# eaymerich/2015-RayTracing

Hardware: AMD Instinct MI355X
Metric: Msamples/sec (pixels x spp) at 1920x1080 (higher is better)
Workload: dtype f32; 1 GPU; A10 cornell.xml path trace 1920x1080, 256 spp (16x16 lens grid), 1 pass, 8 bounces, thin lens; one fused launch that resolves its own pixels (mirt_render_first_pass, no per-ray accumulator); width=1920, height=1080, rays_per_pixel=256, bounces=8, parallelism=rows/1, workload_key=cornell_1920x1080_r256_b8_n1

## Files before the change

2015-raytracing_amd/csrc/mirt_abi.cpp:

```cpp
#include "../../include/mirt.h"
#include "pt_launch.hpp"
#include "pt_post_check.hpp"
#include "pt_rows_plan.hpp"
#include "pt_view_plan.hpp"
#include "pt_set_guard.hpp"
#include "pt_stream_match.hpp"
#include "pt_upsample_taps.hpp"

#include <hip/hip_runtime.h>
#include <dlfcn.h>

#include <algorithm>
#include <cctype>
#include <cmath>
#include <cstdarg>
#include <cstdio>
#include <cstdlib>
#include <cstring>
#include <mutex>
#include <string>
#include <atomic>
#include <unordered_map>
#include <unordered_set>
#include <vector>

namespace {

constexpr size_t kRayBytes = 48, kPoiBytes = 64, kAcuBytes = 16;

thread_local std::string t_last_error = "";

enum HandleKind : uint8_t { H_CTX = 1, H_BUF, H_KERNEL, H_GRAPH, H_GROUP };
std::mutex g_live_mu;
std::unordered_map<const void*, HandleKind> g_live;
std::atomic<uint64_t> g_next_uid{1};

void live_add(const void* p, HandleKind k) { std::lock_guard<std::mutex> l(g_live_mu); g_live[p] = k; }
void live_del(const void* p) { std::lock_guard<std::mutex> l(g_live_mu); g_live.erase(p); }
bool live_is(const void* p, HandleKind k) {
    if (!p) return false;
    std::lock_guard<std::mutex> l(g_live_mu);
    auto it = g_live.find(p);
    return it != g_live.end() && it->second == k;
}

}

struct mirt_graph;
struct mirt_group;

using pt::ArgType; using pt::A_BUF; using pt::KernelId; using pt::KernelSpec; using pt::KArg; using pt::Enqueue; using pt::kKernels; using pt::arg_size; using pt::f2u_host;

struct mirt_ctx {
    int device = -1;
    hipStream_t own_stream = nullptr;
    hipStream_t stream = nullptr;
    std::string last_error;
    void* scratch = nullptr;
// ... 18 lines not shown
    size_t view_defer_bytes = 0;
    uint32_t view_defer_words = 0;
    bool inpass_resolve = true;
    bool last_pass_resolved = false;
    int force_exact = 0;
    bool profiling = false;
    hipEvent_t pe[3] = {nullptr, nullptr, nullptr};
    bool pe_valid = false;
    bool capturing = false;
    std::unordered_set<mirt_buf*> bufs;
    std::unordered_set<mirt_kernel*> kernels;
    std::unordered_set<mirt_graph*> graphs;
    mirt_group* group = nullptr;
    int fusion = 0;
    std::vector<Enqueue> pending;
    uint64_t fused_passes = 0;
    uint64_t guided_passes = 0;
    bool frame_fusion = false;
    uint64_t fused_frames = 0;
    uint64_t scratch_gen = 1, defer_gen = 1;
    struct Pin { mirt_buf* buf; uint64_t uid; uint64_t prep_gen; uint64_t version; bool content; };
    std::vector<Pin> cap_pins;
    bool cap_scratch = false, cap_defer = false;
};

static int flush_pending(mirt_ctx* ctx);
#define FLUSH_PENDING(ctx) do { if (!(ctx)->pending.empty()) { int _rc = flush_pending(ctx); if (_rc) return _rc; } } while (0)

struct mirt_graph {
    mirt_ctx* ctx = nullptr;
    hipGraph_t graph = nullptr;
    hipGraphExec_t exec = nullptr;
    std::vector<mirt_ctx::Pin> pins;
    uint64_t scratch_gen = 0, defer_gen = 0;
};

struct mirt_buf {
    mirt_ctx* ctx = nullptr;
    void* ptr = nullptr;
    size_t bytes = 0;
    bool owned = true;
    unsigned flags = 0;
    uint64_t uid = 0;
    uint64_t version = 1;
    uint64_t off_version = 0;
    uint32_t off_n = 0;
    uint32_t off_last = 0;
    uint32_t prep_count = 0;
    void* prep = nullptr;
    size_t prep_bytes = 0;
    uint64_t prep_version = 0;
    uint64_t prep_gen = 1;
    bool prep_sane = false;
};

struct mirt_kernel {
    mirt_ctx* ctx = nullptr;
    const KernelSpec* spec = nullptr;
    std::vector<KArg> args;
};

namespace {

bool live_has(const mirt_ctx* p) { return live_is(p, H_CTX); }
bool live_has(const mirt_buf* p) { return live_is(p, H_BUF); }
bool live_has(const mirt_kernel* p) { return live_is(p, H_KERNEL); }
bool live_has(const mirt_graph* p) { return live_is(p, H_GRAPH); }

int fail(mirt_ctx* ctx, int code, const char* fmt, ...) {
    char buf[512];
    va_list ap;
    va_start(ap, fmt);
    vsnprintf(buf, sizeof buf, fmt, ap);
    va_end(ap);
    t_last_error = buf;
    if (ctx && live_has(ctx)) ctx->last_error = buf;
    return code;
}

#define HIPCHK(ctx, expr)                                                                          \
    do {                                                                                           \
        hipError_t _e = (expr);                                                                    \
        if (_e != hipSuccess) return fail((ctx), MIRT_E_DEVICE, "%s: %s", #expr, hipGetErrorString(_e)); \
    } while (0)

#define NOT_WHILE_CAPTURING(ctx, what) \
    do { if ((ctx)->capturing) return fail((ctx), MIRT_E_ARG, "%s is not possible inside mirt_capture_begin/end: run the sequence once before recording it", (what)); } while (0)

void pin(mirt_ctx* ctx, const mirt_buf* b, bool content) {
    if (!ctx->capturing) return;
    for (auto& p : ctx->cap_pins)
        if (p.buf == b) { p.content = p.content || content; return; }
    ctx->cap_pins.push_back({const_cast<mirt_buf*>(b), b->uid, b->prep_gen, b->version, content});
}

int need(mirt_ctx* ctx, const char* what, const mirt_buf* b, uint64_t bytes) {
    if (!live_has(b)) return fail(ctx, MIRT_E_HANDLE, "%s: released or unknown buffer", what);
    if (b->ctx != ctx) return fail(ctx, MIRT_E_ARG, "%s: buffer belongs to another context", what);
    if ((uint64_t)b->bytes < bytes)
        return fail(ctx, MIRT_E_RANGE, "%s: buffer holds %zu bytes, launch needs %llu", what, b->bytes, (unsigned long long)bytes);
    pin(ctx, b, false);
    return MIRT_OK;
}

int check_grid(mirt_ctx* ctx, const char* what, mirt_buf* off, uint32_t n, const mirt_buf* prims, size_t prim_stride,
               const mirt_buf* normals, const mirt_buf* matid) {
    if (n == 0 || n > 1024) return fail(ctx, MIRT_E_ARG, "%s: n_slabs %u outside 1..1024", what, n);
    const uint64_t cells = (uint64_t)n * n * n;
    int rc = need(ctx, what, off, (cells + 1) * 4);
    if (rc) return rc;
    if (!off->owned || !(off->off_version == off->version && off->off_n == n)) {
        NOT_WHILE_CAPTURING(ctx, "validating a new cell-offset table");
        std::vector<uint32_t> h(cells + 1);
        HIPCHK(ctx, hipMemcpyAsync(h.data(), off->ptr, (cells + 1) * 4, hipMemcpyDeviceToHost, ctx->stream));
        HIPCHK(ctx, hipStreamSynchronize(ctx->stream));
        for (uint64_t i = 0; i < cells; ++i) {
            if (h[i] > h[i + 1]) return fail(ctx, MIRT_E_DATA, "%s: cell offsets decrease at cell %llu", what, (unsigned long long)i);
            if (n > 1 && h[i + 1] - h[i] >= pt::kMaxCellSlots)
                return fail(ctx, MIRT_E_RANGE, "%s: cell %llu holds %u slots (a cell of a grid holds at most %u)", what, (unsigned long long)i, h[i + 1] - h[i], pt::kMaxCellSlots - 1u);
        }
        off->off_version = off->version;
        off->off_n = n;
        off->off_last = h[cells];
    }
    pin(ctx, off, true);
    const uint64_t count = off->off_last;
    rc = need(ctx, what, prims, count * prim_stride);
    if (rc) return rc;
    if (normals && (rc = need(ctx, what, normals, count * prim_stride))) return rc;
    if (matid && (rc = need(ctx, what, matid, count * 4))) return rc;
    return MIRT_OK;
}

int ensure_scratch(mirt_ctx* ctx, size_t bytes);

int ensure_prepared(mirt_ctx* ctx, mirt_buf* pb, uint32_t count) {
    const size_t bytes = pt::prepared_bytes(count);
    if (pb->owned && pb->prep_version == pb->version && pb->prep_count == count && pb->prep_bytes >= bytes && (pb->prep || !bytes)) { pin(ctx, pb, true); return MIRT_OK; }
    NOT_WHILE_CAPTURING(ctx, "preparing a new triangle buffer");
    if (pb->prep && pb->prep_bytes < bytes) { HIPCHK(ctx, hipStreamSynchronize(ctx->stream)); HIPCHK(ctx, hipFree(pb->prep)); pb->prep = nullptr; pb->prep_bytes = 0; pb->prep_gen++; }
    if (bytes && !pb->prep) { HIPCHK(ctx, hipMalloc(&pb->prep, bytes)); pb->prep_bytes = bytes; pb->prep_gen++; }
    int rc = ensure_scratch(ctx, 16);
    if (rc) return rc;
    uint32_t insane = 0;
    HIPCHK(ctx, hipMemsetAsync(ctx->scratch, 0, 4, ctx->stream));
    pt::launch_prepTriangles(ctx->stream, pb->ptr, pb->prep, count, (uint32_t*)ctx->scratch);
    HIPCHK(ctx, hipMemcpyAsync(&insane, ctx->scratch, 4, hipMemcpyDeviceToHost, ctx->stream));
    HIPCHK(ctx, hipStreamSynchronize(ctx->stream));
    pb->prep_sane = insane == 0;
    pb->prep_version = pb->version;
    if (pb->prep_count != count) pb->prep_gen++;
    pb->prep_count = count;
    return MIRT_OK;
}

int ensure_scratch(mirt_ctx* ctx, size_t bytes) {
    if (ctx->capturing) ctx->cap_scratch = true;
    if (ctx->scratch_bytes >= bytes) return MIRT_OK;
    NOT_WHILE_CAPTURING(ctx, "growing the scratch buffer");
    if (ctx->scratch) { HIPCHK(ctx, hipStreamSynchronize(ctx->stream)); HIPCHK(ctx, hipFree(ctx->scratch)); ctx->scratch = nullptr; ctx->scratch_bytes = 0; }
    ctx->scratch_gen++;
    HIPCHK(ctx, hipMalloc(&ctx->scratch, bytes));
    ctx->scratch_bytes = bytes;
    return MIRT_OK;
}

int grow_and_clear(mirt_ctx* ctx, void*& ptr, size_t& have, size_t need_bytes) {
    if (have < need_bytes) {
        if (ptr) { HIPCHK(ctx, hipStreamSynchronize(ctx->stream)); HIPCHK(ctx, hipFree(ptr)); ptr = nullptr; have = 0; }
        HIPCHK(ctx, hipMalloc(&ptr, need_bytes));
        have = need_bytes;
    }
    HIPCHK(ctx, hipMemsetAsync(ptr, 0, need_bytes, ctx->stream));
    return MIRT_OK;
}

void add_range(std::vector<pt::PostRange>& in, const mirt_buf* b) { if (b && live_has(b)) in.push_back({(uint64_t)(uintptr_t)b->ptr, (uint64_t)b->bytes, true}); }
void add_geometry_ranges(std::vector<pt::PostRange>& in, const mirt_pass_desc* d) {
    const auto add_grid = [&in](const mirt_grid* g) { if (g) { add_range(in, g->prims); add_range(in, g->normals); add_range(in, g->matid); add_range(in, g->cell_offsets); } };
    add_grid(d->spheres); add_grid(d->triangles);
    for (uint32_t m = 0; m < d->n_meshes; ++m) add_grid(&d->meshes[m]);
}

void free_buf(mirt_buf* buf, bool ctx_alive) {
    mirt_ctx* ctx = buf->ctx;
    live_del(buf);
    if (ctx_alive) {
        ctx->bufs.erase(buf);
        if ((buf->owned && buf->ptr) || buf->prep) {
            (void)hipSetDevice(ctx->device);
            (void)hipStreamSynchronize(ctx->stream);
        }
        if (buf->owned && buf->ptr) (void)hipFree(buf->ptr);
        if (buf->prep) (void)hipFree(buf->prep);
    }
    delete buf;
}
void free_kernel(mirt_kernel* k, bool ctx_alive) {
    live_del(k);
    if (ctx_alive) k->ctx->kernels.erase(k);
    delete k;
}
// ... 847 lines not shown
            if ((rc = need(ctx, "pixels", A(K::pixels), npx * 4))) return rc;
            if ((rc = need(ctx, "rays", A(K::rays), npx * kRayBytes))) return rc;
            if (S.id == pt::K_a04_initTrace) pt::launch_frame_initTrace(st, false, A(K::pixels)->ptr, A(K::fcam), A(K::rays)->ptr, nullptr, g0, g1);
            else if (S.id == pt::K_a07_initTrace) pt::launch_frame_initTrace(st, true, A(K::pixels)->ptr, A(K::fcam), A(K::rays)->ptr, A(pt::a07_initTrace::bound), g0, g1);
            else {
                namespace M4 = pt::a04_meshTrace; namespace MM = pt::a07_molTrace; namespace MT = pt::a07_meshTrace;
                pt::FrameArgs F = {};
                memcpy(F.cam, A(K::fcam), 64); F.pixels = A(K::pixels)->ptr; F.rays = A(K::rays)->ptr; F.gx = g0; F.gy = g1;
                if (S.id == pt::K_a04_meshTrace) rc = frame_a04_mesh(ctx, S.name, A(M4::t_size), A(M4::t_pos), A(M4::t_normal), A(M4::t_mindex), A(M4::m_color), F);
                else if (S.id == pt::K_a07_molTrace) rc = frame_a07_mol(ctx, S.name, A(MM::bound), A(MM::n_slabs), A(MM::slab_size), A(MM::s_atoms), F);
                else rc = frame_a07_mesh(ctx, S.name, A(MT::bound), A(MT::n_slabs), A(MT::slab_size), A(MT::t_pos), A(MT::t_normal), F);
                if (rc) return rc;
                pt::launch_frame_stage(st, F, S.id == pt::K_a04_meshTrace ? pt::FS_A04 : S.id == pt::K_a07_molTrace ? pt::FS_MOL : pt::FS_MESH);
            }
            break;
        }
        default:
            return fail(ctx, MIRT_E_NAME, "kernel not implemented");
    }
    HIPCHK(ctx, hipGetLastError());
    return MIRT_OK;
}

static int fill_grid(mirt_ctx* ctx, const char* what, const mirt_grid* g, bool tri, bool per_prim_matid, pt::GridArgs* o) {
    if (!g->prims || !g->cell_offsets) return fail(ctx, MIRT_E_ARG, "%s: null geometry buffer", what);
    if (tri && !g->normals) return fail(ctx, MIRT_E_ARG, "%s: triangles need a normal buffer", what);
    if (per_prim_matid && !g->matid) return fail(ctx, MIRT_E_ARG, "%s: needs a per-primitive material buffer", what);
    int rc = check_grid(ctx, what, g->cell_offsets, g->n_slabs, g->prims, tri ? 48 : 16, tri ? g->normals : nullptr,
                        per_prim_matid ? g->matid : nullptr);
    if (rc) return rc;
    o->prims = g->prims->ptr;
    o->kind = tri ? pt::KIND_TRIANGLES : pt::KIND_SPHERES;
    if (tri) {
        mirt_buf* pb = g->prims;
        if ((rc = ensure_prepared(ctx, pb, g->cell_offsets->off_last))) return rc;
        o->prims = pb->prep ? pb->prep : pb->ptr;
        o->pnorm = pb->prep && g->cell_offsets->off_last <= pt::kLdsTriMax ? (const char*)pb->prep + pt::prepared_planes_offset(g->cell_offsets->off_last) : nullptr;
    }
    o->normals = tri ? g->normals->ptr : nullptr;
    o->matid = per_prim_matid ? g->matid->ptr : nullptr;
    o->off = g->cell_offsets->ptr;
    memcpy(o->bound, g->bounds, sizeof o->bound);
    o->n = g->n_slabs;
    o->mesh_matid = g->mesh_matid;
    o->nslots = g->cell_offsets->off_last;
    const pt::SetGuard v = pt::set_guard(g->bounds, g->n_slabs, !tri || g->prims->prep_sane);
    o->fast_ok = v.fast_ok;
    o->walk_ok = v.walk_ok;
    o->exit_is_far_face = v.exit_is_far_face;
    o->exit_far_axes = v.exit_far_axes;
    memcpy(o->exit_up, v.exit_up, sizeof o->exit_up);
    memcpy(o->delta, v.delta, sizeof o->delta);
    memcpy(o->rdelta, v.rdelta, sizeof o->rdelta);
    return MIRT_OK;
}

static pt::PassRequest pass_request(const mirt_ctx* ctx, const mirt_pass_desc* d, const PassOpts& o) {
    pt::PassRequest r;
    r.rpp = d->rays_per_pixel;
    r.npix = (uint64_t)(d->nrows ? d->nrows : d->height) * d->width;
    r.passes = o.passes;
    r.fresh = o.fresh;
    r.has_acu = d->acu != nullptr;
    r.has_pixel = d->pixel != nullptr;
    r.has_radiance = d->radiance != nullptr;
    r.every = o.every;
    r.inpass_resolve = ctx->inpass_resolve;
    return r;
}

static int fill_sets(mirt_ctx* ctx, const char* fn, const mirt_pass_desc* d, pt::FusedArgs& A);
static int fill_shading(mirt_ctx* ctx, const mirt_pass_desc* d, pt::FusedArgs& A, bool with_material);
static int pass_setup(mirt_ctx* ctx, const char* fn, const mirt_pass_desc* d, bool guides, pt::FusedArgs& A, bool with_material = true) {
    if (!d || d->struct_size != sizeof(mirt_pass_desc)) return fail(ctx, MIRT_E_ARG, "%s: descriptor size mismatch", fn);
    if (!d->width || !d->height || !d->rays_per_pixel) return fail(ctx, MIRT_E_ARG, "%s: empty image", fn);
    {
        const uint32_t k = (uint32_t)std::sqrt((double)d->rays_per_pixel);
        const uint32_t kk = (k + 1) * (k + 1) == d->rays_per_pixel ? k + 1 : k;
        if (kk * kk != d->rays_per_pixel)
            return fail(ctx, MIRT_E_ARG, "%s: rays_per_pixel %u is not a square (the lens grid is k x k, A10 code.js:540)", fn, d->rays_per_pixel);
    }
    if (!guides && d->n_lights > MIRT_MAX_LIGHTS) return fail(ctx, MIRT_E_ARG, "%s: %u lights > %d (enqueue the kernels one by one instead)", fn, d->n_lights, MIRT_MAX_LIGHTS);
    if (d->n_meshes > MIRT_MAX_MESHES) return fail(ctx, MIRT_E_ARG, "%s: %u meshes > %d (enqueue the kernels one by one instead)", fn, d->n_meshes, MIRT_MAX_MESHES);
    if ((!guides && d->n_lights && !d->lights) || (d->n_meshes && !d->meshes)) return fail(ctx, MIRT_E_ARG, "%s: null light/mesh array", fn);
    if (!guides && !d->pass_index) return fail(ctx, MIRT_E_ARG, "%s: pass_index is 1-based", fn);
    const uint32_t cols = f2u_host(d->cam[14]), rows = f2u_host(d->cam[15]);
    if (cols != d->width || rows != d->height) return fail(ctx, MIRT_E_ARG, "%s: camera says %ux%u, descriptor %ux%u", fn, cols, rows, d->width, d->height);
    const uint32_t nrows = d->nrows ? d->nrows : d->height;
    if (d->row0 >= d->height || nrows > d->height - d->row0) return fail(ctx, MIRT_E_ARG, "%s: row tile [%u,+%u) outside the image", fn, d->row0, nrows);
    const uint64_t npix = (uint64_t)nrows * d->width;
    const uint64_t nrays = npix * d->rays_per_pixel;
    if (nrays > 0xFFFFFF00ull) return fail(ctx, MIRT_E_ARG, "%s: %llu rays in one tile (the kernels index a tile's rays with 32 bits); split the rows over more launches", fn, (unsigned long long)nrays);
    HIPCHK(ctx, hipSetDevice(ctx->device));

    memset(&A, 0, sizeof A);
    memcpy(A.cam, d->cam, sizeof A.cam);
    memcpy(A.bound, d->scene_bounds, sizeof A.bound);
    A.focal_length = d->focal_length; A.lens_rad = d->lens_rad;
    A.width = d->width; A.height = d->height; A.rpp = d->rays_per_pixel;
    A.row0 = d->row0; A.nrows = nrows; A.bounces = d->bounces;
    A.n_lights = guides ? 0u : d->n_lights;
    int rc;
    if ((rc = fill_sets(ctx, fn, d, A))) return rc;
    return fill_shading(ctx, d, A, with_material);
}

// ... 1391 lines not shown
```

2015-raytracing_amd/csrc/pt_direct.hpp:

```cpp
#pragma once
#include "pt_closest.hpp"

#ifndef PT_SKIP_DARK_SHADOWS
#define PT_SKIP_DARK_SHADOWS 1
#endif
namespace pt {

template <int STRIDE, bool ATTE_LDS>
struct ParkT : ClosestHooks {
    static constexpr bool kAtteLds = ATTE_LDS;
    static constexpr int kP = ATTE_LDS ? 7 : 4, kN = kP + 3;
    float* base;
    PT_DEV void put(int w, float v) const { base[w * STRIDE] = v; }
    PT_DEV float get(int w) const { return base[w * STRIDE]; }
    PT_DEV void acc_add(float x, float y, float z) const {
        put(0, get(0) + x); put(1, get(1) + y); put(2, get(2) + z); put(3, get(3) + 1.0f);
    }
    PT_DEV void put_pn(const Poi& q) const { put(kP, q.p.x); put(kP + 1, q.p.y); put(kP + 2, q.p.z); put(kN, q.n.x); put(kN + 1, q.n.y); put(kN + 2, q.n.z); }
    PT_DEV void get_pn(Poi& q) const { q.p = mk3(get(kP), get(kP + 1), get(kP + 2)); q.n = mk3(get(kN), get(kN + 1), get(kN + 2)); }
};
typedef ParkT<256, true> Park;

template <bool FAST, int GRIDS, class PARK>
PT_DEV void direct_all(const FusedArgs& A, Poi& poi, int32_t& seed, float4& acc, const PARK& park, bool& defer) {
    const float4* material = (const float4*)A.material;
    for (uint32_t l = 0; l < A.n_lights; ++l) {
        const LightArgs& L = A.lights[l];
        const bool path = poi.matId >= 0;
        bool dark = false;
        Ray sh;
        sh.o = mk3(0.0f, 0.0f, 0.0f);
        sh.d = mk3(0.0f, 0.0f, 0.0f);
        sh.mint = PT_INF;
        sh.maxt = PT_INF;
        if (path) {
#if PT_PARK_LDS
            if (PT_PARK_PN_FOR(GRIDS)) park.get_pn(poi);
#endif
            sh = shadow_ray(poi, ld3(L.shadow), ld3(L.shadow + 3), ld3(L.shadow + 6), L.shadow[9], seed);
#if PT_SKIP_DARK_SHADOWS
            if (GRIDS) {
                const float cosx = cl_clamp(dot3(sh.d, poi.n), 0.0f, 1.0f);
                const float cosy = cl_clamp(dot3(neg3(sh.d), ld3(L.scene + 3)), 0.0f, 1.0f);
                const float r = len3(sub3(poi.p, ld3(L.scene)));
                const float fin = L.scene[9] * 0.0f + L.scene[6] * 0.0f + L.scene[7] * 0.0f + L.scene[8] * 0.0f;
                dark = (cosx * cosy == 0.0f) & (r * r > 0.0f) & (fin == 0.0f);
            }
            if (FAST && !dark) defer = defer || !ray_guard(sh);
#else
            if (FAST) defer = defer || !ray_guard(sh);
#endif
        }
        const RayRcp rr = ray_rcp<FAST>(sh);
        for (uint32_t s = 0; s < A.n_sets; ++s) {
            const GridArgs& S = A.sets[s];
            const bool live = path && !dark && !(sh.mint == sh.maxt);
            Hit ch;
            bool walked = false;
            if (!GRIDS || S.n == 1u) {
                if (live) {
                    pt_count(PC_BOX_TESTS); pt_count(PC_BOX_LANES, true);
                    const BoxHit bh = inter_aabb_t<FAST, !PT_AABB_UNSIGNED_ZERO>(sh, rr, set_box(S));
                    if (bh.v) {
                        ch = (S.kind == KIND_SPHERES) ? trace_cell1<SPHERES, true, TRI_A10, FAST, true>(sh, rr, bh, S) : trace_cell1<TRIANGLES, true, TRI_A10, FAST, true, PT_LANE_LISTS_FOR(FAST, GRIDS)>(sh, rr, bh, S);
                        walked = true;
                    }
                }
            } else if (S.kind == KIND_TRIANGLES) {
                BoxHit bh = {};
                if (live) bh = inter_aabb_t<FAST, true>(sh, rr, set_box(S));
                walked = live && bh.v;
                ch = trace_dda_coop<COOP_ANY, FAST, GRIDS == 1>(walked, sh, rr, bh, S, defer);
            } else if (live) {
                const BoxHit bh = inter_aabb_t<FAST, true>(sh, rr, set_box(S));
                if (bh.v) {
                    ch = trace_dda<SPHERES, true, TRI_A10, FAST, GRIDS == 1>(sh, bh, S, defer);
                    walked = true;
                }
            }
            if (!walked) continue;
            sh.maxt = ch.t;
            if (ch.idx != UINT32_MAX) sh.mint = ch.t;
        }
        if (!path || (uint32_t)poi.matId >= A.nmat) continue;
        pt_count(PC_SHADE); pt_count(PC_SHADE_LANES, true);
        float4 c4 = material[poi.matId];
#if PT_PARK_LDS
        if (PT_PARK_PN_FOR(GRIDS)) park.get_pn(poi);
        if (PARK::kAtteLds) poi.atte = mk3(park.get(4), park.get(5), park.get(6));
        f3 c = shade_vertex(poi, sh, mk3(c4.x, c4.y, c4.z), ld3(L.scene), ld3(L.scene + 3), ld3(L.scene + 6), L.scene[9]);
        if (PARK::kAtteLds) { park.put(4, poi.atte.x); park.put(5, poi.atte.y); park.put(6, poi.atte.z); }
        park.acc_add(c.x, c.y, c.z);
#else
        f3 c = shade_vertex(poi, sh, mk3(c4.x, c4.y, c4.z), ld3(L.scene), ld3(L.scene + 3), ld3(L.scene + 6), L.scene[9]);
        acc.x += c.x; acc.y += c.y; acc.z += c.z; acc.w += 1.0f;
#endif
    }
}

}
```

2015-raytracing_amd/csrc/pt_launch.hpp:

```cpp
#pragma once
#include <hip/hip_runtime.h>
#include <stdint.h>

#include "pt_pass_plan.hpp"

namespace pt {

enum { KIND_SPHERES = 0, KIND_TRIANGLES = 1 };

void launch_sizeof(hipStream_t s, bool ray, uint32_t* out);
void launch_initAcu(hipStream_t s, void* acu, uint32_t total, uint32_t gsz);
void launch_lensDraws(hipStream_t s, void* seeds, void* uv, uint32_t cols, uint32_t rows, uint32_t gx, uint32_t gy,
                      uint32_t row0, uint32_t nrows);
void launch_initTrace(hipStream_t s, void* rays, void* pois, const void* uv, const float* bound, const float* cam,
                      float focal, float lens_rad, uint32_t rpp, uint32_t gx, uint32_t gy);
void launch_bouncePaths(hipStream_t s, const void* pois, void* rays, void* seeds, uint32_t total, uint32_t gsz);
void launch_lightRender(hipStream_t s, void* pois, void* rays, void* acu, const float* light, uint32_t total, uint32_t gsz);
void launch_initShadowTrace(hipStream_t s, void* shadow, const void* pois, uint32_t total, const float* light, void* seeds, uint32_t gsz);
void launch_closest(hipStream_t s, int kind, uint32_t total, void* pois, void* rays, const void* prims, const void* normals,
                    const void* matid, uint32_t mesh_matid, const void* off, const float* bound, uint32_t n, uint32_t exit_far, uint32_t gsz);
void launch_anyhit(hipStream_t s, int kind, uint32_t total, void* shadow, const void* prims, const void* off, const float* bound,
                   uint32_t n, uint32_t exit_far, uint32_t gsz);
void launch_sceneRender(hipStream_t s, void* acu, void* pois, const void* shadow, const void* material, uint32_t nmat,
                        const float* light, uint32_t total, uint32_t gsz);
void launch_copyToPixel(hipStream_t s, void* pixel, const void* acu, float m, uint32_t pixels, uint32_t rpp, uint32_t gsz, void* radiance);
void launch_numerics(hipStream_t s, int op, const void* a, const void* b, void* out, uint64_t n);
void launch_divCheck(hipStream_t s, int mode, uint64_t seed, uint64_t count, void* out16);
void launch_seedFill(hipStream_t s, void* seeds, uint64_t first, uint64_t count, uint32_t base);

constexpr int kMaxLights = 8;
constexpr int kMaxMeshes = 16;

constexpr uint32_t kNoLds = 0xFFFFFFFFu;
constexpr uint32_t kLdsOffWords = 4096;
constexpr uint32_t kLdsTriMax = 96;
struct GridArgs {
    const void* prims;
    const void* pnorm;
    const void* normals;
    const void* matid;
    const void* off;
    float bound[8];
    uint32_t n;
    uint32_t mesh_matid;
    uint32_t kind;
    uint32_t fast_ok;
    uint32_t lds_off;
    float delta[3], rdelta[3];
    uint32_t nslots;
    uint32_t exit_far_axes;
    float exit_up[3];
    uint32_t walk_ok;
    uint32_t exit_is_far_face;
};
struct LightArgs {
    float shadow[16];
    float scene[16];
    float light[16];
};
struct FusedArgs {
    float cam[16];
    float bound[8];
    float focal_length, lens_rad;
    uint32_t width, height, rpp;
    uint32_t row0, nrows;
    uint32_t bounces;
    uint32_t n_sets, n_lights;
    GridArgs sets[2 + kMaxMeshes];
    LightArgs lights[kMaxLights];
    const void* material;
    uint32_t nmat;
    int32_t* seeds;
    void* acu;
    const void* uv;
    uint32_t fresh;
    void* pixel;
    void* radiance;
    float res_m;
    uint32_t resolve;
    uint32_t seg_off;
    uint32_t seg_len;
    uint32_t seg_pitch;
    uint32_t passes;
    uint32_t every;
    uint32_t pass_index;
    const void* carry;
    void* guide_nh;
    void* guide_ad;
};
inline bool all_sets_fast_ok(const FusedArgs& a) { for (uint32_t i = 0; i < a.n_sets; ++i) if (!a.sets[i].fast_ok) return false; return true; }
void launch_fused(hipStream_t s, const FusedArgs& a, bool fast, uint32_t* defer_mask, const uint32_t* redo_mask, uint32_t redo_words);
bool fused_fast_available();
bool fused_has_grids(const FusedArgs& a);
bool fused_multipass_default(const FusedArgs& a);
void launch_deferCount(hipStream_t s, const uint32_t* mask, uint32_t words, uint32_t* count);
void launch_guides(hipStream_t s, const FusedArgs& a, bool fast, void* normal_hits, void* albedo_depth, uint32_t* defer_mask, const uint32_t* redo_mask);
void launch_rays(hipStream_t s, const FusedArgs& a, bool fast, const void* rays, uint32_t count, void* hits, uint32_t* sets, uint8_t* occluded,
                 uint32_t* defer_mask, const uint32_t* redo_mask);
void launch_ao(hipStream_t s, const FusedArgs& a, bool fast, uint32_t samples, float radius, float bias, void* ao_out, uint32_t* defer_mask, const uint32_t* redo_mask);
void launch_radiance(hipStream_t s, const FusedArgs& a, bool fast, const void* rays, uint32_t count, uint32_t samples, uint32_t flags, int32_t* seeds, void* radiance,
                     uint32_t* defer_mask, const uint32_t* redo_mask);
struct ViewArgs {
    uint32_t model;
    uint32_t width, height;
    uint32_t k;
    uint32_t row0, nrows;
// ... 99 lines not shown
```

2015-raytracing_amd/csrc/pt_trace.hpp:

```cpp
#pragma once
#include "pt_device.hpp"
#include "pt_launch.hpp"
#include "pt_windows.hpp"

#ifndef PT_UNROLL_UNIFORM
#define PT_UNROLL_UNIFORM 1
#endif

namespace pt {

#ifndef PT_COUNT
#define PT_COUNT 0
#endif
enum PtCounter { PC_WAVES = 0, PC_SEGMENTS, PC_SEG_LANES, PC_Q_CLOSEST, PC_Q_CLOSEST_LANES, PC_SWEEP_CLOSEST, PC_TRIPS_CLOSEST, PC_TRIP_LANES_CLOSEST,
                 PC_Q_SHADOW, PC_Q_SHADOW_LANES, PC_SWEEP_SHADOW, PC_TRIPS_SHADOW, PC_TRIP_LANES_SHADOW,
                 PC_SPH_Q_CLOSEST, PC_SPH_Q_CLOSEST_LANES, PC_SPH_TESTS_CLOSEST, PC_SPH_ROOTS_CLOSEST, PC_SPH_Q_SHADOW, PC_SPH_Q_SHADOW_LANES, PC_SPH_TESTS_SHADOW, PC_SPH_ROOTS_SHADOW,
                 PC_BOX_TESTS, PC_BOX_LANES, PC_SHADE, PC_SHADE_LANES, PC_BOUNCE, PC_BOUNCE_LANES,
                 PC_GRID_WALKS, PC_GRID_WANT_LANES = PC_GRID_WALKS + 2, PC_GRID_PHASES = PC_GRID_WALKS + 4, PC_GRID_A_STEPS = PC_GRID_WALKS + 6,
                 PC_GRID_A_LANE_STEPS = PC_GRID_WALKS + 8, PC_GRID_ROUNDS = PC_GRID_WALKS + 10, PC_GRID_PAIRS = PC_GRID_WALKS + 12, PC_COUNT = 48 };
#if PT_COUNT
static __device__ unsigned long long pt_counters[PC_COUNT];
__device__ __forceinline__ void pt_count(int i, bool lanes = false, unsigned long long n = 1ull) {
    const unsigned long long m = __builtin_amdgcn_ballot_w64(true);
    const unsigned me = __builtin_amdgcn_mbcnt_hi(~0u, __builtin_amdgcn_mbcnt_lo(~0u, 0u));
    if (me == (unsigned)__builtin_ctzll(m)) atomicAdd(&pt_counters[i], lanes ? (unsigned long long)__builtin_popcountll(m) : n);
}
#else
__device__ __forceinline__ void pt_count(int, bool = false, unsigned long long = 1ull) {}
#endif

struct Hit { uint32_t idx; float t, beta, gamma; };

PT_DEV f3 interp_normal(const float4* nn, float beta, float gamma) {
    const float w = 1.0f - beta - gamma;
    return norm3(fma3(gamma, ld3(nn[2]), fma3(w, ld3(nn[0]), scl3(beta, ld3(nn[1])))));
}

#define PT_CONST_AS __attribute__((address_space(4)))
typedef float pt_v4f __attribute__((ext_vector_type(4)));
typedef float pt_v16f __attribute__((ext_vector_type(16)));
PT_DEV float4 ldc4(const void* base, size_t idx) {
    const pt_v4f v = ((const pt_v4f PT_CONST_AS*)base)[idx];
    return make_float4(v.x, v.y, v.z, v.w);
}
PT_DEV uint32_t ldc_u32(const void* base, size_t idx) { return ((const uint32_t PT_CONST_AS*)base)[idx]; }

#ifndef PT_GUARD_INT
#define PT_GUARD_INT 1
#endif
enum TriRule { TRI_A10 = 0, TRI_A07 = 1, TRI_A04 = 2 };
#ifndef PT_UNIFORM_CULL
#define PT_UNIFORM_CULL 0
#endif
#ifndef PT_SPHERE_WAVE_SKIP
#define PT_SPHERE_WAVE_SKIP 1
#endif
template <int RULE = TRI_A10, bool FAST = false, bool WAVE_CULL = false>
PT_DEV bool tri_test(f3 o, f3 d, float cmin, float cmax, const float4 A, const float4 B, const float4 C,
                     float& t_out, float& beta_out, float& gamma_out) {
    const f3 p0 = mk3(A.x, A.y, A.z), e1 = mk3(B.x, B.y, B.z), e2 = mk3(C.x, C.y, C.z), n = mk3(A.w, B.w, C.w);
    float div = dot3(n, d);
    if (WAVE_CULL && __builtin_amdgcn_ballot_w64(!(div <= 0)) == 0ull) { t_out = 0.0f; beta_out = 0.0f; gamma_out = 0.0f; return false; }
    float idiv;
    if (FAST) idiv = rcp_refined(div);
    else idiv = rcp_plain(div);
    f3 s = sub3(o, p0);
    float beta = dot3(cross3(s, d), e2) * idiv;
    float gamma = dot3(cross3(s, e1), d) * idiv;
    float gb = gamma + beta;
    float t = dot3(cross3(s, e2), e1) * -idiv;
    int ok = !(div <= 0);
    ok &= !(beta < 0.0f) & !(beta > 1.0f);
// ... 192 lines not shown
    const bool fwd = d >= 0;
    a.dslab = fwd ? 1 : -1;
    a.limit = fwd ? (int)n : -1;
    a.dt = div_exact3_anyzero(delta, cl_fabs(d), cl_fabs(rd));
    const float xnext = cl_fma((float)(a.slab + (fwd ? 1 : 0)), delta, lo);
    const float num1 = xnext - o;
    a.tnext = div_exact3_anyzero(num1, d, rd);
    defer = ((int)defer | (int)!((int)num_window(num0) & (int)num_window(num1))) != 0;
    return a;
}

PT_DEV uint32_t sign_word(float w) {
    uint32_t r;
    asm("v_ashrrev_i32 %0, 31, %1" : "=v"(r) : "v"(w));
    return r;
}

extern __shared__ __attribute__((aligned(16))) uint32_t pt_lds_dyn[];

PT_DEV Box set_box_of(const GridArgs& S) {
    Box b;
    b.lo = mk3(S.bound[0], S.bound[1], S.bound[2]);
    b.hi = mk3(S.bound[4], S.bound[5], S.bound[6]);
    return b;
}
template <bool FAST>
PT_DEV float cell1_exit(const Ray& ray, const RayRcp& rr, const BoxHit& bh, const GridArgs& S) {
    float tn[3];
    if (S.exit_is_far_face) {
        tn[0] = bh.tfx; tn[1] = bh.tfy; tn[2] = bh.tfz;
#if !PT_PLAIN_DIV
    } else if (FAST) {
        const float tf[3] = {bh.tfx, bh.tfy, bh.tfz}, up[3] = {S.exit_up[0], S.exit_up[1], S.exit_up[2]};
        const float oo[3] = {ray.o.x, ray.o.y, ray.o.z}, dd[3] = {ray.d.x, ray.d.y, ray.d.z}, rc[3] = {rr.x, rr.y, rr.z};
#pragma unroll
        for (int k = 0; k < 3; ++k) {
            const float q = div_exact3_anyzero(up[k] - oo[k], dd[k], rc[k]);
            tn[k] = (((S.exit_far_axes >> k) & 1u) != 0u || !(dd[k] >= 0.0f)) ? tf[k] : q;
        }
#endif
    } else {
        const float lo[3] = {S.bound[0], S.bound[1], S.bound[2]}, hi[3] = {S.bound[4], S.bound[5], S.bound[6]};
        const float oo[3] = {ray.o.x, ray.o.y, ray.o.z}, dd[3] = {ray.d.x, ray.d.y, ray.d.z};
#pragma unroll
        for (int k = 0; k < 3; ++k) {
            float delta = (hi[k] - lo[k]) / 1.0f;
            float xnext = lo[k] + (float)((dd[k] >= 0) ? 1 : 0) * delta;
            tn[k] = (xnext - oo[k]) / dd[k];
        }
    }
    return cl_min(cl_min(tn[0], tn[1]), tn[2]);
}

template <int KIND, bool ANY, int RULE = TRI_A10, bool FAST = false, bool FLAG_ONLY = false, bool LANES = false>
PT_DEV Hit trace_cell1(const Ray& ray, const RayRcp& rr, const BoxHit& bh, const GridArgs& S) {
    Hit ch;
    ch.idx = UINT32_MAX;
    ch.t = ray.maxt;
    ch.beta = 0.0f;
    ch.gamma = 0.0f;
    SphereRay sr;
    if (KIND == SPHERES) sr = sphere_ray<FAST>(ray.d);
    const float cmin = bh.tmin;
    const float cmax = cell1_exit<FAST>(ray, rr, bh, S);
    const uint32_t begin = __builtin_amdgcn_readfirstlane(ldc_u32(S.off, 0));
    const uint32_t end = __builtin_amdgcn_readfirstlane(ldc_u32(S.off, 1));
    bool done = false;
    if (LANES && KIND == TRIANGLES && FAST && RULE == TRI_A10 && S.lds_off != kNoLds && begin == 0u) {
        const pt_v16f PT_CONST_AS* pn = (const pt_v16f PT_CONST_AS*)((const char PT_CONST_AS*)S.pnorm + 64);
        const uint32_t lds_bytes = S.lds_off * 4u;
        const float o1 = __builtin_fabsf(ray.o.x) + __builtin_fabsf(ray.o.y) + __builtin_fabsf(ray.o.z);
        const float hi_p = __builtin_fmaxf(__builtin_fminf(cmax, ray.maxt) * 1.00000095367431640625f, 0x1p-100f);
        const float lo_m = cmin * 0.99999904632568359375f;
        pt_count(ANY ? PC_Q_SHADOW : PC_Q_CLOSEST); pt_count(ANY ? PC_Q_SHADOW_LANES : PC_Q_CLOSEST_LANES, true);
        for (uint32_t c0 = 0u; c0 < end; c0 += 32u) {
            const uint32_t groups = ldc_u32(S.pnorm, c0 >> 5);
            const pt_v16f PT_CONST_AS* g = pn + ldc_u32(S.pnorm, 4u + (c0 >> 5));
            const float Mu = cl_fma(__uint_as_float(ldc_u32(S.pnorm, 8u + (c0 >> 5))), o1, __uint_as_float(ldc_u32(S.pnorm, 12u + (c0 >> 5))));
            uint32_t cand = 0u;
            auto verdict = [&](float div, float sn, uint32_t mask, uint32_t back) {
                const float sp = sn + Mu, sm = sn - Mu;
                const float w = __builtin_fminf(__builtin_fminf(div, cl_fma(hi_p, div, sp)), -cl_fma(lo_m, div, sm));
                cand |= mask & ~sign_word(w);
                if (back != 0u) {
                    asm volatile("" ::: "memory");
                    const float wb = __builtin_fminf(__builtin_fminf(-div, -cl_fma(hi_p, div, sm)), cl_fma(lo_m, div, sp));
                    cand |= back & ~sign_word(wb);
                }
            };
#define PT_AXIS_GROUPS(SHIFT, OA, DA)                                                                                   \
            for (uint32_t i = 0; i < ((groups >> SHIFT) & 255u); ++i, ++g) {                                            \
                const pt_v16f v = *g;                                                                                   \
                _Pragma("unroll") for (int k = 0; k < 4; ++k) {                                                         \
                    const uint32_t mask = __float_as_uint(v[4 * k + 2]), back = __float_as_uint(v[4 * k + 3]);          \
                    if ((mask | back) == 0u) continue;                 \
                    asm volatile("" ::: "memory");                                                                      \
                    pt_count(ANY ? PC_SWEEP_SHADOW : PC_SWEEP_CLOSEST);                                                 \
                    verdict(v[4 * k + 1] * (DA), v[4 * k + 1] * ((OA) - v[4 * k]), mask, back);                         \
                }                                                                                                       \
            }
            PT_AXIS_GROUPS(0, ray.o.x, ray.d.x)
            PT_AXIS_GROUPS(8, ray.o.y, ray.d.y)
            PT_AXIS_GROUPS(16, ray.o.z, ray.d.z)
#undef PT_AXIS_GROUPS
            for (uint32_t i = 0; i < groups >> 24; ++i, ++g) {
                const pt_v16f v = *g;
#pragma unroll
                for (int k = 0; k < 2; ++k) {
                    const uint32_t mask = __float_as_uint(v[8 * k + 4]), back = __float_as_uint(v[8 * k + 5]);
                    if ((mask | back) == 0u) continue;
                    asm volatile("" ::: "memory");
                    pt_count(ANY ? PC_SWEEP_SHADOW : PC_SWEEP_CLOSEST);
                    const float div = dot3(mk3(v[8 * k], v[8 * k + 1], v[8 * k + 2]), ray.d);
                    const float sn = cl_fma(v[8 * k + 2], ray.o.z, cl_fma(v[8 * k + 1], ray.o.y, cl_fma(v[8 * k], ray.o.x, -v[8 * k + 3])));
                    verdict(div, sn, mask, back);
                }
            }
            if (ANY && done) cand = 0u;
            while (cand != 0u) {
                pt_count(ANY ? PC_TRIPS_SHADOW : PC_TRIPS_CLOSEST); pt_count(ANY ? PC_TRIP_LANES_SHADOW : PC_TRIP_LANES_CLOSEST, true);
                const uint32_t k = (uint32_t)__builtin_clz(cand);
                cand &= ~(0x80000000u >> k);
                const uint32_t i = c0 + k;
                const float4* __restrict__ q = (const float4*)((const char*)pt_lds_dyn + (lds_bytes + __umul24(i, 48u)));
                float ti, b, gm;
                const bool hit = tri_test_nn(ray.o, ray.d, cmin, cmax, q[0], q[1], q[2], ti, b, gm);
                if (ANY && FLAG_ONLY) {
                    if (hit && ti < ray.maxt) { done = true; cand = 0u; }
                    continue;
                }
                const bool better = (int)hit & (int)(ti < ch.t);
                ch.t = better ? ti : ch.t;
                ch.idx = better ? i : ch.idx;
                ch.beta = better ? b : ch.beta;
                ch.gamma = better ? gm : ch.gamma;
                if (ANY && better) { done = true; cand = 0u; }
            }
            if (ANY && __builtin_amdgcn_ballot_w64(!done) == 0ull) break;
        }
        if (ANY && FLAG_ONLY && done) ch.idx = 0u;
        return ch;
    }
    if (KIND == SPHERES) { pt_count(ANY ? PC_SPH_Q_SHADOW : PC_SPH_Q_CLOSEST); pt_count(ANY ? PC_SPH_Q_SHADOW_LANES : PC_SPH_Q_CLOSEST_LANES, true); }
    const pt_v4f PT_CONST_AS* p = (const pt_v4f PT_CONST_AS*)S.prims + (size_t)begin * (KIND == SPHERES ? 1u : 3u);
#if PT_UNROLL_UNIFORM > 1
#pragma unroll PT_UNROLL_UNIFORM
#endif
    for (uint32_t i = begin; i < end; ++i, p += (KIND == SPHERES ? 1 : 3)) {
        float ti, b = 0.0f, gm = 0.0f;
        bool hit;
        if (KIND == SPHERES) {
            pt_count(ANY ? PC_SPH_TESTS_SHADOW : PC_SPH_TESTS_CLOSEST);
            hit = sph_test<FAST, PT_SPHERE_WAVE_SKIP != 0, ANY ? PC_SPH_ROOTS_SHADOW : PC_SPH_ROOTS_CLOSEST>(ray.o, ray.d, sr, cmin, cmax, ldc4((const void*)p, 0), ti);
        } else {
            hit = tri_test<RULE, FAST, PT_UNIFORM_CULL != 0>(ray.o, ray.d, cmin, cmax, ldc4((const void*)p, 0), ldc4((const void*)p, 1), ldc4((const void*)p, 2), ti, b, gm);
        }
// ... 115 lines not shown
```

profiles/trip_counts.py:

```python
#!/usr/bin/env python3
import ctypes as C
import json
import os
import sys

import numpy as np

ROOT = os.path.dirname(os.path.dirname(os.path.abspath(__file__)))
sys.path.insert(0, ROOT)
import __graft_entry__ as graft

NAMES = ["waves", "segments", "seg_lanes", "q_closest", "q_closest_lanes", "sweep_closest", "trips_closest", "trip_lanes_closest",
         "q_shadow", "q_shadow_lanes", "sweep_shadow", "trips_shadow", "trip_lanes_shadow",
         "sph_q_closest", "sph_q_closest_lanes", "sph_tests_closest", "sph_roots_closest", "sph_q_shadow", "sph_q_shadow_lanes", "sph_tests_shadow", "sph_roots_shadow",
         "box_tests", "box_lanes", "shade", "shade_lanes", "bounce", "bounce_lanes",
         "grid_walks_closest", "grid_walks_shadow", "grid_want_lanes_closest", "grid_want_lanes_shadow", "grid_phases_closest", "grid_phases_shadow",
         "grid_a_steps_closest", "grid_a_steps_shadow", "grid_a_lane_steps_closest", "grid_a_lane_steps_shadow", "grid_rounds_closest", "grid_rounds_shadow",
         "grid_pairs_closest", "grid_pairs_shadow"]


def main():
    graft.load_package()
    from raytracing_amd.pyhost import mirt, render, scene
    name = sys.argv[1] if len(sys.argv) > 1 else "cornell"
    w, h, rpp, bounces = (int(x) for x in (sys.argv[2:6] if len(sys.argv) > 5 else (1920, 1080, 16, 8)))
    if name == "cornell":
        base = scene.PackedScene(open(os.path.join(ROOT, "tests", "golden", "scene_cornell_1920x1080_r256.json")).read())
    else:
        fx = np.load(os.path.join(ROOT, "tests", "golden", name + ".npz"))
        base = scene.PackedScene(bytes(fx["scene_json"]).decode())
    sc = base.resized(w, h, rpp)
    lib = mirt.lib()
    if not hasattr(lib, "mirt_debug_counters"):
        raise SystemExit("this libmirt.so is not a counting build (-DPT_COUNT=1)")
    ctx = mirt.Context(0)
    fr = render.FusedRenderer(ctx, sc, keep_acu=False)
    out = (C.c_ulonglong * 48)()
    lib.mirt_debug_counters(None, 1)
    fr.execute_render(bounces=bounces, fresh=True)
    ctx.finish()
    lib.mirt_debug_counters(out, 0)
    c = dict(zip(NAMES, list(out)))
    waves = c["waves"]
    print(json.dumps({"scene": name, "width": w, "height": h, "rpp": rpp, "bounces": bounces, "counters": c}))
    print(f"{'counter':28s} {'total':>14s} {'per wave':>10s}")
    for k in NAMES:
        print(f"{k:28s} {c[k]:14d} {c[k] / waves:10.2f}")
    fr.release()
    ctx.destroy()


if __name__ == "__main__":
    main()
```

Before: 5530 Msamples/s.

## Skip axis-aligned plane tests for shadow rays inside a precomputed empty gap

Adds a host-side analysis of the axis-aligned triangle planes of a single-cell triangle set. It computes a conservative slab on each axis that no axis-aligned plane crosses, with error margins. In the shadow path, a wave whose rays all have segments inside that slab skips the AABB test and all axis-aligned plane groups, and tests only the general-plane groups. This adds a plane readback at prep time and a per-ray gap test with a wave ballot, at the risk of extra divergence or of the test rarely passing.

```diff
diff --git a/2015-raytracing_amd/csrc/mirt_abi.cpp b/2015-raytracing_amd/csrc/mirt_abi.cpp
--- a/2015-raytracing_amd/csrc/mirt_abi.cpp
+++ b/2015-raytracing_amd/csrc/mirt_abi.cpp
@@ -4,6 +4,7 @@
 #include "pt_rows_plan.hpp"
 #include "pt_view_plan.hpp"
 #include "pt_set_guard.hpp"
+#include "pt_shadow_gap.hpp"
 #include "pt_stream_match.hpp"
 #include "pt_upsample_taps.hpp"
 
@@ -128,6 +129,8 @@
     uint64_t prep_version = 0;
     uint64_t prep_gen = 1;
     bool prep_sane = false;
+    bool gap_planes_ok = false;
+    pt::GapPlanes gap_planes;
 };
 
 struct mirt_kernel {
@@ -222,8 +225,14 @@
     HIPCHK(ctx, hipMemsetAsync(ctx->scratch, 0, 4, ctx->stream));
     pt::launch_prepTriangles(ctx->stream, pb->ptr, pb->prep, count, (uint32_t*)ctx->scratch);
     HIPCHK(ctx, hipMemcpyAsync(&insane, ctx->scratch, 4, hipMemcpyDeviceToHost, ctx->stream));
+    std::vector<uint32_t> planes;
+    if (count && count <= pt::kLdsTriMax) {
+        planes.resize(pt::prepared_planes_bytes(count) / 4);
+        HIPCHK(ctx, hipMemcpyAsync(planes.data(), (const char*)pb->prep + pt::prepared_planes_offset(count), planes.size() * 4, hipMemcpyDeviceToHost, ctx->stream));
+    }
     HIPCHK(ctx, hipStreamSynchronize(ctx->stream));
     pb->prep_sane = insane == 0;
+    pb->gap_planes_ok = !planes.empty() && pt::gap_planes_from_list(planes.data(), (uint32_t)planes.size(), count, &pb->gap_planes) != 0;
     pb->prep_version = pb->version;
     if (pb->prep_count != count) pb->prep_gen++;
     pb->prep_count = count;
@@ -1177,6 +1186,13 @@
     memcpy(o->exit_up, v.exit_up, sizeof o->exit_up);
     memcpy(o->delta, v.delta, sizeof o->delta);
     memcpy(o->rdelta, v.rdelta, sizeof o->rdelta);
+    o->gap_ok = 0u;
+    memset(o->gap, 0, sizeof o->gap);
+    if (tri && o->pnorm && g->n_slabs == 1u && v.fast_ok && g->prims->gap_planes_ok && g->prims->prep_count == g->cell_offsets->off_last) {
+        const pt::ShadowGap sg = pt::shadow_gap(g->bounds, v.exit_up, &g->prims->gap_planes, 1.0);
+        memcpy(o->gap, sg.qlo, 12); memcpy(o->gap + 3, sg.qhi, 12); memcpy(o->gap + 6, sg.gm, 12); memcpy(o->gap + 9, sg.hm, 12);
+        o->gap_ok = sg.ok;
+    }
     return MIRT_OK;
 }
 
diff --git a/2015-raytracing_amd/csrc/pt_direct.hpp b/2015-raytracing_amd/csrc/pt_direct.hpp
--- a/2015-raytracing_amd/csrc/pt_direct.hpp
+++ b/2015-raytracing_amd/csrc/pt_direct.hpp
@@ -4,7 +4,25 @@
 #ifndef PT_SKIP_DARK_SHADOWS
 #define PT_SKIP_DARK_SHADOWS 1
 #endif
+#ifndef PT_SHADOW_GAP
+#define PT_SHADOW_GAP 1
+#endif
+#define PT_SHADOW_GAP_FOR(FAST, GRIDS) (PT_SHADOW_GAP && (GRIDS) == 0 && PT_LANE_LISTS_FOR(FAST, GRIDS))
 namespace pt {
+
+PT_DEV bool gap_test(const Ray& r, const float* gap) {
+    const float o1 = __builtin_fabsf(r.o.x) + __builtin_fabsf(r.o.y) + __builtin_fabsf(r.o.z);
+    const float hi_p = __builtin_fmaxf(r.maxt * 1.00000095367431640625f, 0x1p-100f);
+    const float oo[3] = {r.o.x, r.o.y, r.o.z}, dd[3] = {r.d.x, r.d.y, r.d.z};
+    int pass = 1;
+#pragma unroll
+    for (int a = 0; a < 3; ++a) {
+        const float e = cl_fma(hi_p, dd[a], oo[a]);
+        const float m = cl_fma(gap[6 + a], o1, gap[9 + a]);
+        pass &= (int)(__builtin_fminf(oo[a], e) - gap[a] > m) & (int)(gap[3 + a] - __builtin_fmaxf(oo[a], e) > m);
+    }
+    return pass != 0;
+}
 
 template <int STRIDE, bool ATTE_LDS>
 struct ParkT : ClosestHooks {
@@ -59,11 +77,25 @@
             bool walked = false;
             if (!GRIDS || S.n == 1u) {
                 if (live) {
-                    pt_count(PC_BOX_TESTS); pt_count(PC_BOX_LANES, true);
-                    const BoxHit bh = inter_aabb_t<FAST, !PT_AABB_UNSIGNED_ZERO>(sh, rr, set_box(S));
-                    if (bh.v) {
-                        ch = (S.kind == KIND_SPHERES) ? trace_cell1<SPHERES, true, TRI_A10, FAST, true>(sh, rr, bh, S) : trace_cell1<TRIANGLES, true, TRI_A10, FAST, true, PT_LANE_LISTS_FOR(FAST, GRIDS)>(sh, rr, bh, S);
+                    bool gap = false;
+                    if (PT_SHADOW_GAP_FOR(FAST, GRIDS) && S.gap_ok != 0u && S.lds_off != kNoLds) {
+                        const bool pass = gap_test(sh, S.gap);
+                        gap = __builtin_amdgcn_ballot_w64(!pass) == 0ull;
+                        pt_count(PC_GAP_ASKED);
+                        if (gap) pt_count(PC_GAP_TAKEN);
+                        if (PT_COUNT && !pass) pt_count(PC_GAP_REFUSED_LANES, true);
+                    }
+                    if (gap) {
+                        BoxHit bh = {};
+                        ch = trace_cell1<TRIANGLES, true, TRI_A10, FAST, true, PT_LANE_LISTS_FOR(FAST, GRIDS), true>(sh, rr, bh, S);
                         walked = true;
+                    } else {
+                        pt_count(PC_BOX_TESTS); pt_count(PC_BOX_LANES, true);
+                        const BoxHit bh = inter_aabb_t<FAST, !PT_AABB_UNSIGNED_ZERO>(sh, rr, set_box(S));
+                        if (bh.v) {
+                            ch = (S.kind == KIND_SPHERES) ? trace_cell1<SPHERES, true, TRI_A10, FAST, true>(sh, rr, bh, S) : trace_cell1<TRIANGLES, true, TRI_A10, FAST, true, PT_LANE_LISTS_FOR(FAST, GRIDS)>(sh, rr, bh, S);
+                            walked = true;
+                        }
                     }
                 }
             } else if (S.kind == KIND_TRIANGLES) {
diff --git a/2015-raytracing_amd/csrc/pt_launch.hpp b/2015-raytracing_amd/csrc/pt_launch.hpp
--- a/2015-raytracing_amd/csrc/pt_launch.hpp
+++ b/2015-raytracing_amd/csrc/pt_launch.hpp
@@ -52,6 +52,8 @@
     float exit_up[3];
     uint32_t walk_ok;
     uint32_t exit_is_far_face;
+    uint32_t gap_ok;
+    float gap[12];
 };
 struct LightArgs {
     float shadow[16];
diff --git a/2015-raytracing_amd/csrc/pt_shadow_gap.hpp b/2015-raytracing_amd/csrc/pt_shadow_gap.hpp
--- /dev/null
+++ b/2015-raytracing_amd/csrc/pt_shadow_gap.hpp
@@ -0,0 +1,84 @@
+#pragma once
+#include <math.h>
+#include <stdint.h>
+#include <string.h>
+
+#ifdef __cplusplus
+namespace pt {
+#endif
+
+enum { kGapMaxPlanes = 96 };
+
+typedef struct GapPlanes {
+    uint32_t n[3];
+    float q[3][kGapMaxPlanes];
+    double g[3], h[3];
+} GapPlanes;
+
+typedef struct ShadowGap {
+    float qlo[3], qhi[3], gm[3], hm[3];
+    uint32_t ok;
+} ShadowGap;
+
+static inline float gap_word_float(uint32_t w) { float f; memcpy(&f, &w, 4); return f; }
+
+static inline int gap_planes_from_list(const uint32_t* words, uint32_t n_words, uint32_t count, GapPlanes* out) {
+    memset(out, 0, sizeof *out);
+    if (n_words < 16u || count == 0u || count > (uint32_t)kGapMaxPlanes) return 0;
+    for (uint32_t c = 0; c < (count + 31u) / 32u; ++c) {
+        const uint32_t groups = words[c], first = words[4u + c];
+        const float G = gap_word_float(words[8u + c]), H = gap_word_float(words[12u + c]);
+        uint32_t g = 16u + 16u * first;
+        for (uint32_t cl = 0; cl < 3u; ++cl) {
+            for (uint32_t i = 0; i < ((groups >> (8u * cl)) & 255u); ++i, g += 16u) {
+                if (g + 16u > n_words) return 0;
+                for (uint32_t k = 0; k < 4u; ++k) {
+                    const uint32_t* e = words + g + 4u * k;
+                    if ((e[2] | e[3]) == 0u) continue;
+                    const float na = fabsf(gap_word_float(e[1]));
+                    if (out->n[cl] >= (uint32_t)kGapMaxPlanes || !(na > 0.0f)) return 0;
+                    out->q[cl][out->n[cl]++] = gap_word_float(e[0]);
+                    out->g[cl] = fmax(out->g[cl], (double)G / (double)na);
+                    out->h[cl] = fmax(out->h[cl], (double)H / (double)na);
+                }
+            }
+        }
+    }
+    return 1;
+}
+
+static inline float gap_round_up(double v) {
+    float f = (float)v;
+    if ((double)f < v) f = nextafterf(f, INFINITY);
+    return f;
+}
+
+static inline ShadowGap shadow_gap(const float* b8, const float* exit_up, const GapPlanes* P, double scale) {
+    ShadowGap s;
+    memset(&s, 0, sizeof s);
+    int ok = 1;
+    for (int a = 0; a < 3; ++a) {
+        const float lo = b8[a], top = fminf(b8[4 + a], exit_up[a]);
+        const float c = 0.5f * lo + 0.5f * b8[4 + a];
+        float qlo = lo, qhi = top;
+        for (uint32_t i = 0; i < P->n[a]; ++i) {
+            const float q = P->q[a][i];
+            if (q <= c && q > qlo) qlo = q;
+            if (q > c && q < qhi) qhi = q;
+        }
+        ok = ok && lo <= c && c < top && qlo < qhi && b8[4 + a] >= top && exit_up[a] >= top;
+        const double Q = fmax(fabs((double)qlo), fabs((double)qhi));
+        s.qlo[a] = qlo;
+        s.qhi[a] = qhi;
+        s.gm[a] = gap_round_up(P->g[a] * 1.0625 * 1.0000019073486328125 * scale);
+        s.hm[a] = gap_round_up((P->h[a] * 1.0625 + 0x1p-23 * Q) * 1.0000019073486328125 * scale);
+        ok = ok && isfinite(s.qlo[a]) && isfinite(s.qhi[a]) && isfinite(s.gm[a]) && isfinite(s.hm[a]) && s.hm[a] >= 0x1p-120f &&
+             (double)qhi - (double)qlo > 2.0 * (double)s.hm[a];
+    }
+    s.ok = ok ? 1u : 0u;
+    return s;
+}
+
+#ifdef __cplusplus
+}
+#endif
diff --git a/2015-raytracing_amd/csrc/pt_trace.hpp b/2015-raytracing_amd/csrc/pt_trace.hpp
--- a/2015-raytracing_amd/csrc/pt_trace.hpp
+++ b/2015-raytracing_amd/csrc/pt_trace.hpp
@@ -17,7 +17,8 @@
                  PC_SPH_Q_CLOSEST, PC_SPH_Q_CLOSEST_LANES, PC_SPH_TESTS_CLOSEST, PC_SPH_ROOTS_CLOSEST, PC_SPH_Q_SHADOW, PC_SPH_Q_SHADOW_LANES, PC_SPH_TESTS_SHADOW, PC_SPH_ROOTS_SHADOW,
                  PC_BOX_TESTS, PC_BOX_LANES, PC_SHADE, PC_SHADE_LANES, PC_BOUNCE, PC_BOUNCE_LANES,
                  PC_GRID_WALKS, PC_GRID_WANT_LANES = PC_GRID_WALKS + 2, PC_GRID_PHASES = PC_GRID_WALKS + 4, PC_GRID_A_STEPS = PC_GRID_WALKS + 6,
-                 PC_GRID_A_LANE_STEPS = PC_GRID_WALKS + 8, PC_GRID_ROUNDS = PC_GRID_WALKS + 10, PC_GRID_PAIRS = PC_GRID_WALKS + 12, PC_COUNT = 48 };
+                 PC_GRID_A_LANE_STEPS = PC_GRID_WALKS + 8, PC_GRID_ROUNDS = PC_GRID_WALKS + 10, PC_GRID_PAIRS = PC_GRID_WALKS + 12,
+                 PC_GAP_ASKED = PC_GRID_WALKS + 14, PC_GAP_TAKEN, PC_GAP_REFUSED_LANES, PC_COUNT = 48 };
 #if PT_COUNT
 static __device__ unsigned long long pt_counters[PC_COUNT];
 __device__ __forceinline__ void pt_count(int i, bool lanes = false, unsigned long long n = 1ull) {
@@ -316,7 +317,7 @@
     return cl_min(cl_min(tn[0], tn[1]), tn[2]);
 }
 
-template <int KIND, bool ANY, int RULE = TRI_A10, bool FAST = false, bool FLAG_ONLY = false, bool LANES = false>
+template <int KIND, bool ANY, int RULE = TRI_A10, bool FAST = false, bool FLAG_ONLY = false, bool LANES = false, bool GAP = false>
 PT_DEV Hit trace_cell1(const Ray& ray, const RayRcp& rr, const BoxHit& bh, const GridArgs& S) {
     Hit ch;
     ch.idx = UINT32_MAX;
@@ -325,8 +326,8 @@
     ch.gamma = 0.0f;
     SphereRay sr;
     if (KIND == SPHERES) sr = sphere_ray<FAST>(ray.d);
-    const float cmin = bh.tmin;
-    const float cmax = cell1_exit<FAST>(ray, rr, bh, S);
+    const float cmin = GAP ? 0.0f : bh.tmin;
+    const float cmax = GAP ? ray.maxt : cell1_exit<FAST>(ray, rr, bh, S);
     const uint32_t begin = __builtin_amdgcn_readfirstlane(ldc_u32(S.off, 0));
     const uint32_t end = __builtin_amdgcn_readfirstlane(ldc_u32(S.off, 1));
     bool done = false;
@@ -334,7 +335,7 @@
         const pt_v16f PT_CONST_AS* pn = (const pt_v16f PT_CONST_AS*)((const char PT_CONST_AS*)S.pnorm + 64);
         const uint32_t lds_bytes = S.lds_off * 4u;
         const float o1 = __builtin_fabsf(ray.o.x) + __builtin_fabsf(ray.o.y) + __builtin_fabsf(ray.o.z);
-        const float hi_p = __builtin_fmaxf(__builtin_fminf(cmax, ray.maxt) * 1.00000095367431640625f, 0x1p-100f);
+        const float hi_p = __builtin_fmaxf((GAP ? ray.maxt : __builtin_fminf(cmax, ray.maxt)) * 1.00000095367431640625f, 0x1p-100f);
         const float lo_m = cmin * 0.99999904632568359375f;
         pt_count(ANY ? PC_Q_SHADOW : PC_Q_CLOSEST); pt_count(ANY ? PC_Q_SHADOW_LANES : PC_Q_CLOSEST_LANES, true);
         for (uint32_t c0 = 0u; c0 < end; c0 += 32u) {
@@ -363,9 +364,13 @@
                     verdict(v[4 * k + 1] * (DA), v[4 * k + 1] * ((OA) - v[4 * k]), mask, back);                         \
                 }                                                                                                       \
             }
-            PT_AXIS_GROUPS(0, ray.o.x, ray.d.x)
-            PT_AXIS_GROUPS(8, ray.o.y, ray.d.y)
-            PT_AXIS_GROUPS(16, ray.o.z, ray.d.z)
+            if (GAP) {
+                g += (groups & 255u) + ((groups >> 8) & 255u) + ((groups >> 16) & 255u);
+            } else {
+                PT_AXIS_GROUPS(0, ray.o.x, ray.d.x)
+                PT_AXIS_GROUPS(8, ray.o.y, ray.d.y)
+                PT_AXIS_GROUPS(16, ray.o.z, ray.d.z)
+            }
 #undef PT_AXIS_GROUPS
             for (uint32_t i = 0; i < groups >> 24; ++i, ++g) {
                 const pt_v16f v = *g;
diff --git a/profiles/trip_counts.py b/profiles/trip_counts.py
--- a/profiles/trip_counts.py
+++ b/profiles/trip_counts.py
@@ -16,7 +16,7 @@
          "box_tests", "box_lanes", "shade", "shade_lanes", "bounce", "bounce_lanes",
          "grid_walks_closest", "grid_walks_shadow", "grid_want_lanes_closest", "grid_want_lanes_shadow", "grid_phases_closest", "grid_phases_shadow",
          "grid_a_steps_closest", "grid_a_steps_shadow", "grid_a_lane_steps_closest", "grid_a_lane_steps_shadow", "grid_rounds_closest", "grid_rounds_shadow",
-         "grid_pairs_closest", "grid_pairs_shadow"]
+         "grid_pairs_closest", "grid_pairs_shadow", "gap_asked", "gap_taken", "gap_refused_lanes"]
 
 
 def main():
```

Measured after the change: 5791 Msamples/s, median of 6. 1.05x the previous value.
